# arkworks-rs/gemini

Measured on AMD Instinct MI355X. Metric: BLS12-381 G1 MSM throughput, higher is better.
Workload: dtype u32x12 Montgomery Fq (381-bit integer), u32x8 Fr; 1 GPU; 2^20 G1 MSM per GPU (BASELINE configs[1]: 2^20 G1 MSM on one MI355X); pairs_per_gpu=1048576

## Files before the change

### gemini_amd/capi.py

```python
from __future__ import annotations

import ctypes as C
import os

import numpy as np

_HERE = os.path.dirname(os.path.abspath(__file__))
LIB_PATH = os.environ.get("GM_LIB_PATH") or os.path.join(_HERE, "libgemini_hip.so")

GM_OK = 0
ERRORS = {-1: "GM_EINVAL", -2: "GM_ENOTINIT", -3: "GM_EHANDLE", -4: "GM_EHIP", -5: "GM_ENOMEM", -6: "GM_ESTATE"}

SYMBOLS = [
    "gm_init", "gm_shutdown", "gm_last_error", "gm_abi_version",
    "gm_g1_msm", "gm_g1_bases_register", "gm_g1_bases_free", "gm_g1_bases_len", "gm_g1_bases_download", "gm_g1_bases_precompute", "gm_set_auto_tables", "gm_g1_bases_table_info", "gm_pool_trim", "gm_g1_release_spare_tables", "gm_mem_stats", "gm_mem_reset_peak", "gm_runtime_info", "gm_snark_footprint", "gm_psnark_footprint", "gm_footprint_admit",
    "gm_g1_msm_h", "gm_g1_msm_v", "gm_g1_msm_v_batch", "gm_g1_msm_v_batch_partial", "gm_g1_msm_v_batch_at", "gm_g1_msm_d", "gm_g1_msm_d_partial", "gm_g1_sum",
    "gm_g1_msm_stream_new", "gm_g1_msm_stream_new_h", "gm_g1_msm_stream_add", "gm_g1_msm_stream_finalize", "gm_g1_msm_stream_free", "gm_host_alloc", "gm_host_free",
    "gm_g1_fixed_base_register", "gm_g1_srs_register", "gm_g1_srs_register_segments", "gm_set_msm_window", "gm_set_msm_table_min", "gm_set_msm_affine_levels", "gm_set_msm_split", "gm_set_msm_glv", "gm_set_msm_sort_group", "gm_debug_msm_sort_path", "gm_prof_enable", "gm_prof_read", "gm_prof_read_clock",
    "gm_idx_register", "gm_idx_free", "gm_idx_len", "gm_idx_download", "gm_idx_extend_frequency", "gm_fr_gather", "gm_fr_alg_hash", "gm_fr_plookup_set", "gm_fr_add_scalar", "gm_fr_shift_monic",
    "gm_fr_acc_product", "gm_fr_tensor_range", "gm_fr_tensor_gather", "gm_fr_powers_gather", "gm_fr_alg_hash_from", "gm_fr_powers_range", "gm_fr_plookup_set_block", "gm_fr_shift_block", "gm_fr_product", "gm_fr_acc_product_block",
    "gm_sc_set_shard_rounds", "gm_sc_round_begin_many", "gm_psnark_shard_block", "gm_psnark_shard_level", "gm_psnark_shard_footprint", "gm_psnark_shard_key_new", "gm_psnark_index_sharded", "gm_psnark_new_time_sharded", "gm_snark_new_elastic_sharded",
    "gm_fr_vec_alloc", "gm_fr_vec_free", "gm_fr_vec_len", "gm_fr_vec_upload", "gm_fr_vec_download",
    "gm_fr_vec_fill", "gm_fr_vec_ptr", "gm_fr_vec_set_len",
    "gm_fr_reverse", "gm_fr_stride", "gm_fr_fold", "gm_fr_fold_chain", "gm_fr_powers", "gm_fr_tensor", "gm_fr_hadamard", "gm_fr_ip", "gm_fr_eval_le", "gm_fr_eval_le_batch",
    "gm_fr_lincomb", "gm_fr_scale_into", "gm_fr_scale_into_many", "gm_fr_add_at", "gm_fr_div_vanishing",
    "gm_spm_register", "gm_spm_free", "gm_spm_mul", "gm_spm_shape", "gm_snark_new_time", "gm_snark_new_elastic", "gm_psnark_new_time", "gm_psnark_new_elastic", "gm_psnark_preprocess", "gm_psnark_preprocess_free", "gm_psnark_index", "gm_spm_download",
    "gm_sc_new", "gm_sc_new_v", "gm_sc_new_borrow", "gm_sc_round", "gm_sc_round_begin", "gm_sc_round_end", "gm_sc_fold", "gm_sc_rounds", "gm_sc_final", "gm_sc_free",
    "gm_sc_set_shard", "gm_sc_lens", "gm_sc_download",
    "gm_sp_new", "gm_sp_new_v", "gm_sp_new_borrow", "gm_sp_round", "gm_sp_fold", "gm_sp_rounds", "gm_sp_final", "gm_sp_to_time", "gm_sp_free",
    "gm_sc_set_herring", "gm_hg1_new", "gm_hg1_round", "gm_hg1_fold", "gm_hg1_rounds", "gm_hg1_final", "gm_hg1_free",
    "gm_g2_msm", "gm_g2_bases_register", "gm_g2_bases_free", "gm_g2_bases_len", "gm_g2_bases_download", "gm_g2_msm_h", "gm_g2_msm_v", "gm_g2_msm_d", "gm_g2_sum",
    "gm_hg2_new", "gm_hg2_round", "gm_hg2_fold", "gm_hg2_rounds", "gm_hg2_final", "gm_hg2_free",
    "gm_pairing_multi", "gm_pairing_multi_h", "gm_gt_mul", "gm_gt_pow", "gm_gt_one", "gm_gt_final_exp",
# ... 71 lines not shown
def ensure_init():
    if not _initialised:
        init()


MEM_FIELDS = ("device_total", "device_free", "held", "held_peak", "pool_cached", "in_use", "in_use_peak", "tables", "keys",
              "spare_table_releases", "msm_workspaces", "reserved")


def mem_stats() -> dict:
    out = np.zeros(12, dtype=np.uint64)
    check(load().gm_mem_stats(ptr(out)))
    return {k: int(v) for k, v in zip(MEM_FIELDS, out)}


FOOTPRINT_FIELDS = ("vectors", "workspaces_to_grow", "needed", "available")


def snark_footprint(ck_handle: int, num_constraints: int, elastic: bool = False) -> dict:
    out = np.zeros(4, dtype=np.uint64)
    check(load().gm_snark_footprint(C.c_uint64(ck_handle), C.c_size_t(num_constraints), C.c_int(int(elastic)), ptr(out)))
    return {k: int(v) for k, v in zip(FOOTPRINT_FIELDS, out)}


def psnark_footprint(ck_handle: int, num_variables: int, nnz: int, elastic: int = 0) -> dict:
    out = np.zeros(4, dtype=np.uint64)
    check(load().gm_psnark_footprint(C.c_uint64(ck_handle), C.c_size_t(num_variables), C.c_size_t(nnz), C.c_int(int(elastic)), ptr(out)))
    return {k: int(v) for k, v in zip(FOOTPRINT_FIELDS, out)}


# ... 25 lines not shown
```

### gemini_amd/csrc/capi.hip

```cpp
#include <cstring>
#include <vector>

#include "ctx.hpp"
#include "host_field.hpp"

namespace gm {

static thread_local char g_err[512] = "";
void set_error(const char* fmt, ...) {
  va_list ap;
  va_start(ap, fmt);
  vsnprintf(g_err, sizeof g_err, fmt, ap);
  va_end(ap);
}
int hip_fail(hipError_t e, const char* what, const char* file, int line) {
  set_error("HIP error %d (%s) in %s at %s:%d", (int)e, hipGetErrorString(e), what, file, line);
  return e == hipErrorOutOfMemory ? GM_ENOMEM : GM_EHIP;
}

MemStats& mem_stats() {
  static MemStats* m = new MemStats;
  return *m;
}
void MemStats::note_cached(ptrdiff_t delta) {
// ... 375 lines not shown
  for (auto& kv : C->provers) sc_destroy(kv.second.get());
  for (auto& kv : C->space_provers) sp_destroy(C, kv.second.get());
  for (auto& kv : C->herring) herring_destroy(C, kv.second.get());
  for (auto& kv : C->g2_bases)
    if (kv.second->d) (void)gm::raw_free(kv.second->d);
  for (auto& kv : C->crs) crs_destroy(kv.second.get());
  C->partial_bufs.release_all();
  for (auto& kv : C->indices)
    if (kv.second->d) (void)gm::raw_free(kv.second->d);
  for (auto& kv : C->matrices) {
    if (kv.second->rowptr) (void)gm::raw_free(kv.second->rowptr);
    if (kv.second->cols) (void)gm::raw_free(kv.second->cols);
    if (kv.second->vals) (void)gm::raw_free(kv.second->vals);
  }
  auto release_ws = [](MsmWorkspace& w) {
    for (DevBuf* b : {&w.scalars, &w.counts, &w.offsets, &w.cursor, &w.entries, &w.tmp_entries, &w.sortmeta, &w.buckets, &w.pk[0], &w.pk[1], &w.pp[0],
                      &w.pp[1], &w.rows, &w.cols, &w.planes, &w.misc, &w.lvl_cnt, &w.lvl_pos, &w.lvl_pts[0], &w.lvl_pts[1], &w.lvl_keys[0],
                      &w.lvl_keys[1], &w.lvl_prefix, &w.lvl_lane, &w.lvl_entries, &w.lvl_n})
      b->release();
    for (int k = 0; k < MSM_SLOTS; k++)
      if (w.host_planes[k]) (void)hipHostFree(w.host_planes[k]);
    if (w.have_done_ev) {
      for (int e = 0; e < MSM_SLOTS; e++) (void)hipEventDestroy(w.done_ev[e]);
    }
  };
  release_ws(C->msm);
  g2_workspace_release(C->g2);
  pairing_workspace_release(C->pairing);
  release_ws(C->msm_b);
  if (C->stream_b) (void)hipStreamDestroy(C->stream_b);
  for (int k = 0; k < MSM_SMALL_LANES; k++) {
// ... 280 lines not shown
           "gm_set_msm_sort_group: a block stages %zu .. %zu entries in its LDS (0 = the most), not %zu", MSM_SORT_GROUP_CAP_MIN, MSM_SORT_GROUP_CAP_MAX, cap);
  std::lock_guard<std::recursive_mutex> lk(C->msm_mu);
  C->msm_sort_group = mode;
  C->msm_sort_group_cap = cap;
  return GM_OK;
}

int gm_debug_msm_sort_path(int* out) {
  GM_CTX();
  GM_CHECK(out != nullptr, GM_EINVAL, "gm_debug_msm_sort_path: null output");
  std::lock_guard<std::recursive_mutex> lk(C->msm_mu);
  *out = C->msm_sort_path_last;
  return GM_OK;
}

int gm_set_msm_split(int on) {
  GM_CTX();
#ifndef GM_EXPERIMENTS
  GM_CHECK(on == 0, GM_EINVAL, "gm_set_msm_split: the window-group experiment is not in this build (make EXTRA=-DGM_EXPERIMENTS; DESIGN.md section 8)");
#endif
  C->msm_split = on != 0;
  return GM_OK;
}

int gm_set_msm_affine_levels(int levels) {
  GM_CTX();
  GM_CHECK(levels >= -1 && levels <= 8, GM_EINVAL, "gm_set_msm_affine_levels: %d not in [-1, 8]", levels);
#ifndef GM_EXPERIMENTS
  if (levels == -1) levels = 0;
  GM_CHECK(levels == 0, GM_EINVAL, "gm_set_msm_affine_levels: the affine-level experiment is not in this build (make EXTRA=-DGM_EXPERIMENTS; DESIGN.md section 8)");
// ... 1595 lines not shown
```

### gemini_amd/csrc/ctx.hpp

```cpp
#pragma once
#include <hip/hip_runtime.h>

#include <atomic>
#include <cstdarg>
#include <cstdint>
#include <cstdio>
#include <map>
#include <memory>
#include <mutex>
#include <string>
#include <unordered_map>
#include <vector>

#include "../../include/gemini_hip.h"

namespace gmh {
struct Fq12;
}

namespace gm {

void set_error(const char* fmt, ...);
int hip_fail(hipError_t e, const char* what, const char* file, int line);

// ... 162 lines not shown
};
struct MsmWorkspace;
constexpr size_t MSM_SORT_GROUP_CAP_MAX = (160 * 1024 - 3 * 1024 * 4 - 64) / 4;
constexpr size_t MSM_SORT_GROUP_CAP_MIN = 1024;
struct MsmPending {
  MsmWorkspace* ws = nullptr;
  int slot = 0;
  bool empty = true;
  int Wb = 0, c = 0, m = 0;
  uint32_t nbits = 0, wf[3] = {0, 0, 0};
  size_t plane_off[3] = {0, 0, 0};
  size_t plane_count = 0;
  int multi_levels = 0;
  int multi_W = 0;
  bool sort_compact = false;
};
struct MsmStreamSlot {
  uint8_t *raw = nullptr, *packed = nullptr, *scalars = nullptr;
  size_t raw_cap = 0, packed_cap = 0, scalars_cap = 0;
  hipEvent_t copied;
  bool have_ev = false;
  bool inflight = false;
  MsmPending P;
};
struct MsmStream {
  std::mutex mu;
  size_t chunk = 0, stride = 96;
  int mont = 0;
  uint64_t bases_handle = 0;
  int64_t base0 = 0, next_base = 0, step = 1;
  MsmStreamSlot s[2];
  int cur = 0;
  size_t fill = 0, total = 0;
  hipStream_t copy = nullptr;
  uint64_t acc[18];
  bool acc_set = false;
};

constexpr int MSM_SLOTS = 4;
constexpr int MSM_SMALL_LANES = 6;
struct MsmWorkspace {
  DevBuf scalars, counts, offsets, cursor, entries, tmp_entries, sortmeta, buckets, pk[2], pp[2], rows, cols, planes, misc;
  DevBuf clk;
  DevBuf lvl_cnt, lvl_pos, lvl_pts[2], lvl_keys[2], lvl_prefix, lvl_lane, lvl_entries, lvl_n;
  uint64_t* host_planes[MSM_SLOTS] = {};
  size_t host_planes_cap[MSM_SLOTS] = {};
  hipEvent_t done_ev[MSM_SLOTS];
  hipEvent_t sort_ev, acc_ev;
  bool have_done_ev = false;
};

enum ProfStage { PROF_DIGITS = 0, PROF_SCAN, PROF_SCATTER, PROF_ACC0, PROF_MERGE, PROF_REDUCE, PROF_SC_ROUND, PROF_EXTFREQ, PROF_NSTAGES };
struct Profiler {
  bool on = false;
  int only_stage = -1;
  hipEvent_t ev[2][2 * PROF_NSTAGES];
  bool have_events = false;
// ... 65 lines not shown
  DevBuf fr_scratch;
  uint64_t* host_small = nullptr;
  uint8_t* sc_desc_host = nullptr;
  uint8_t* sc_desc_dev = nullptr;
  hipEvent_t sc_desc_copied[SC_DESC_SLOTS] = {};
  unsigned sc_desc_next = 0;
  uint64_t* host_batch = nullptr;
  size_t host_batch_cap = 0;
  int msm_c_override = 0;
  int msm_glv = 0;
  int msm_split = 0;
  int msm_affine_levels = 0;
  int msm_sort_group = 1;
  size_t msm_sort_group_cap = 0;
  int msm_sort_path_last = 0;
  size_t msm_table_min = (size_t)1 << 17;
  int zero_copy = 3;
  std::atomic<int> msm_busy{0};
  bool auto_tables = true;
  size_t auto_tables_max = 0;
  int cu_count = 256;
};

Context* context();
struct MemStats {
  std::mutex mu;
  std::unordered_map<void*, size_t> sizes;
  size_t live = 0, peak_live = 0;
  size_t cached = 0;
  size_t peak_in_use = 0;
// ... 133 lines not shown
```

### gemini_amd/csrc/msm.hip

```cpp
#include <algorithm>
#include <atomic>
#include <chrono>
#include <condition_variable>
#include <cstdlib>
#include <cstring>
#include <functional>
#include <sched.h>
#include <cstdio>
#include <thread>
#include <vector>

#include "ctx.hpp"
#include "g1.cuh"
#include "host_field.hpp"

namespace gm {

constexpr uint32_t KEY_INV = 0xffffffffu;
constexpr int XYZZ_BYTES = 192;
constexpr int AFF_BYTES = 96;

struct DigitIter {
  uint32_t s[8];
  uint32_t carry;
// ... 1108 lines not shown

#ifdef GM_EXPERIMENTS
#include "msm_levels.inc"
#endif

__global__ __launch_bounds__(64) void k_merge(const uint32_t* __restrict__ keys_in, const uint8_t* __restrict__ pts_in,
                                              uint32_t E, uint32_t* __restrict__ keys_out,
                                              uint8_t* __restrict__ pts_out, uint8_t* __restrict__ buckets,
                                              int final_level) {
  __shared__ __attribute__((aligned(16))) uint8_t lds[128 * XYZZ30_BYTES];
  const int lane = threadIdx.x;
  const uint32_t wave = blockIdx.x;
  const uint32_t s0 = wave * 128u + 2u * lane;
  uint32_t hk = s0 < E ? keys_in[s0] : KEY_INV;
  uint32_t tk = s0 + 1 < E ? keys_in[s0 + 1] : KEY_INV;
  uint32_t hs = 2 * lane, ts = 2 * lane + 1;
  auto copy_rec = [](void* dst, const void* src) {
    const gm_u4v* s = reinterpret_cast<const gm_u4v*>(src);
    gm_u4v* d = reinterpret_cast<gm_u4v*>(dst);
#pragma unroll
    for (int i = 0; i < 13; i++) d[i] = s[i];
  };
  auto add_slots = [&](uint32_t dst_slot, uint32_t src_slot, Acc30& a) {
    Acc30 o;
    acc30_load(a, lds + dst_slot * XYZZ30_BYTES);
    acc30_load(o, lds + src_slot * XYZZ30_BYTES);
    acc30_add(a, o);
  };
  if (hk != KEY_INV) copy_rec(lds + hs * XYZZ30_BYTES, pts_in + (size_t)s0 * XYZZ30_BYTES);
  if (tk != KEY_INV) copy_rec(lds + ts * XYZZ30_BYTES, pts_in + ((size_t)s0 + 1) * XYZZ30_BYTES);
// ... 70 lines not shown
    __syncthreads();
  }
  if (lane == 0) {
    if (final_level) {
      if (hk != KEY_INV) copy_rec(buckets + (size_t)hk * XYZZ30_BYTES, lds + hs * XYZZ30_BYTES);
      if (tk != KEY_INV) copy_rec(buckets + (size_t)tk * XYZZ30_BYTES, lds + ts * XYZZ30_BYTES);
    } else {
      keys_out[2 * (size_t)wave] = hk;
      keys_out[2 * (size_t)wave + 1] = tk;
      if (hk != KEY_INV) copy_rec(pts_out + (size_t)(2 * (size_t)wave) * XYZZ30_BYTES, lds + hs * XYZZ30_BYTES);
      if (tk != KEY_INV) copy_rec(pts_out + (size_t)(2 * (size_t)wave + 1) * XYZZ30_BYTES, lds + ts * XYZZ30_BYTES);
    }
  }
}

enum { GS_STRIDED = 0, GS_PLANE = 1 };
struct GroupSumArgs {
  const uint8_t* in;
  uint8_t* out;
  int mode;
  uint32_t n_out;
  uint32_t per_win;
  uint32_t win_stride;
  uint32_t n_lo, s_hi, s_lo, s_e, len;
  uint32_t nb;
  uint32_t lpo_shift;
  int out_canonical;
  const uint32_t* in_cnt;
};
struct GroupSumJobs {
  GroupSumArgs j[3];
  uint32_t blk_end[3];
  const uint32_t* err_src;
  uint32_t* err_dst;
  const unsigned long long* clk_src;
  const uint32_t* chunked_src;
};

__global__ __launch_bounds__(256) void k_group_sum(GroupSumJobs J) {
  if (J.err_dst && blockIdx.x == 0 && threadIdx.x == 0) {
    *J.err_dst = *J.err_src;
    J.err_dst[1] = J.chunked_src ? *J.chunked_src : 0u;
    if (J.clk_src) {
      unsigned long long* d = reinterpret_cast<unsigned long long*>(J.err_dst + 2);
      d[0] = J.clk_src[0];
      d[1] = J.clk_src[1];
    }
  }
  const int job = blockIdx.x < J.blk_end[0] ? 0 : (blockIdx.x < J.blk_end[1] ? 1 : 2);
  const GroupSumArgs& a = J.j[job];
  const uint32_t blk0 = job == 0 ? 0u : J.blk_end[job - 1];
  const uint8_t* __restrict__ in = a.in;
  uint8_t* __restrict__ out = a.out;
  const uint32_t gt = (blockIdx.x - blk0) * blockDim.x + threadIdx.x;
  const uint32_t lpo = 1u << a.lpo_shift;
  const uint32_t o = gt >> a.lpo_shift, q = gt & (lpo - 1u);
  Acc30 acc;
  acc30_zero(acc);
  const uint32_t* __restrict__ in_cnt = a.in_cnt;
  auto filled = [&](size_t slot) { return in_cnt == nullptr || in_cnt[slot] != 0u; };
  auto add_rec = [&](size_t slot) {
    if (!filled(slot)) return;
// ... 220 lines not shown
  static const size_t c20_min = getenv("GM_MSM_C20_MIN") ? (size_t)strtoull(getenv("GM_MSM_C20_MIN"), nullptr, 10) : ((size_t)7 << 21);
  if (n >= c20_min) return 20;
  if (lg >= 23) return 19;
  static const int c_medium = getenv("GM_MSM_C_MEDIUM") ? atoi(getenv("GM_MSM_C_MEDIUM")) : 0;
  if (c_medium && lg >= 14 && lg <= 17) return c_medium;
  if (lg >= 14) return 16;
  if (lg >= 11) return 8;
  if (lg >= 8) return lg - 4;
  if (lg >= 5) return lg + 1;
  return 4;
}

size_t msm_workspace_held(const MsmWorkspace& ws) {
  size_t b = 0;
  for (const DevBuf* d : {&ws.scalars, &ws.counts, &ws.offsets, &ws.cursor, &ws.entries, &ws.tmp_entries, &ws.sortmeta, &ws.buckets, &ws.pk[0], &ws.pk[1],
                          &ws.pp[0], &ws.pp[1], &ws.rows, &ws.cols, &ws.planes, &ws.misc, &ws.clk})
    b += d->cap;
  return b;
}
size_t msm_workspace_bound(Context* C, const Bases* bases, size_t n) {
  if (n == 0) return 0;
  n = std::min<size_t>(n, (size_t)1 << 26);
  int c = C->msm_c_override ? C->msm_c_override : choose_window(n);
  bool table = false;
  if (bases && !C->msm_c_override && n < ((size_t)1 << ENTRY_W_SHIFT)) {
    if (bases->table && n >= std::max(C->msm_table_min, bases->tab_min)) {
      c = bases->tab_c;
      table = true;
    } else {
      for (const Bases::TableSet& ts : bases->extra)
        if (n >= ts.min_n && n < ts.max_n && n <= ts.n) {
          c = ts.c;
          table = true;
          break;
        }
    }
  }
  const size_t W = (size_t)(256 + c - 1) / (size_t)c;
  const size_t N = n * W, nbuckets = (table ? 1 : W) << (c - 1);
  auto grow = [](size_t b) { return b + b / 8 + 256; };
  const size_t lanes0 = N >= ((size_t)1 << 24) ? 262144 : 131072;
  const size_t L = std::min<size_t>(256, std::max<size_t>(4, (N + lanes0 - 1) / lanes0)) + 1;
  const size_t E1 = 2 * ((N / L + 256 + 255) / 256 * 256), E2 = 2 * ((E1 + 127) / 128);
  size_t b = 2 * grow(N * 8);
  b += grow(nbuckets * XYZZ30_BYTES) + 4 * grow((nbuckets + 8192) * 4);
  b += grow(E1 * 4) + grow(E1 * XYZZ30_BYTES) + grow(E2 * 4) + grow(E2 * XYZZ30_BYTES);
  b += (size_t)W * ((size_t)3 << 14) * XYZZ30_BYTES + ((size_t)16 << 20);
  return b;
}

constexpr size_t MSM_SMALL_N = (size_t)1 << 17;
constexpr size_t MSM_SPLIT_MIN_N = (size_t)1 << 17;
static int msm_run_one(Context* C, const Bases* bases, int64_t first, int64_t step, const void* d_scalars, int mont, size_t n,
                       bool normalize, uint64_t out_jac[18]);

struct MsmStreams {
  hipStream_t sort, acc, tail;
};
struct MsmMulti {
  bool block = false;
  int levels = 0;
// ... 451 lines not shown
  uint64_t Nacc = N;
  for (int l = 0; l < levels; l++) Nacc = Nacc / 2 + 2 * nbuckets + 2;

  static const int L_env = getenv("GM_MSM_L") ? atoi(getenv("GM_MSM_L")) : 0;
  const uint64_t Nacc_all = nparts > 1 ? Nall : Nacc;
  const uint64_t lanes0 = Nacc_all >= ((uint64_t)1 << 24) ? 262144 : 131072;
  static const uint64_t L_cap = getenv("GM_MSM_LCAP") ? (uint64_t)atoi(getenv("GM_MSM_LCAP")) : 256;
  uint32_t L = (uint32_t)std::min<uint64_t>(L_cap, std::max<uint64_t>(4, (Nacc_all + lanes0 - 1) / lanes0));
  if (L_env > 0) L = (uint32_t)L_env;
  L = (L + 1u) & ~1u;
  const uint64_t T0 = (Nacc + L - 1) / L;
  const uint64_t T0pad = (T0 + 255) / 256 * 256;
  const uint64_t E1 = 2 * T0pad;

  int rc;
  const size_t counts_words = (nbuckets + 2 + SORT_GMAX + 2 + 63) / 64 * 64;
  if ((rc = ws.counts.ensure(counts_words * 4))) return rc;
  if ((rc = ws.offsets.ensure((nbuckets + 1) * 4))) return rc;
  if ((rc = ws.cursor.ensure((nbuckets + 1) * 4))) return rc;
  if ((rc = ws.misc.ensure((nbuckets / SCAN_PER_BLOCK + 2) * 4))) return rc;
  if ((rc = ws.entries.ensure(N * 8))) return rc;
  if ((rc = ws.buckets.ensure(nbuckets * bucket_bytes))) return rc;
  if ((rc = ws.pk[0].ensure(E1 * 4))) return rc;
  if ((rc = ws.pp[0].ensure(E1 * bucket_bytes))) return rc;
  const uint64_t E2 = 2 * ((E1 + 127) / 128);
  if ((rc = ws.pk[1].ensure(E2 * 4))) return rc;
  if ((rc = ws.pp[1].ensure(E2 * bucket_bytes))) return rc;

  const uint32_t* sc = reinterpret_cast<const uint32_t*>(d_scalars);
  GM_HIP(hipMemsetAsync(ws.counts.p, 0, counts_words * 4, st));
  uint32_t* d_err = ws.counts.as<uint32_t>() + nbuckets + 1;
  uint32_t* d_chunked = ws.counts.as<uint32_t>() + nbuckets + 2 + SORT_GMAX + 1;
  const bool bucket_counts_valid = levels == 0;
  if (!bucket_counts_valid) GM_HIP(hipMemsetAsync(ws.buckets.p, 0, nbuckets * bucket_bytes, st));
  const uint32_t dblocks = (uint32_t)((n + 255) / 256);
  Profiler& pf = C->prof;
  auto run_scan = [&]() {
    const uint32_t nb = (uint32_t)((nbuckets + SCAN_PER_BLOCK - 1) / SCAN_PER_BLOCK);
    hipLaunchKernelGGL(k_scan_block_sums, dim3(nb), dim3(256), 0, st, ws.counts.as<uint32_t>(), (uint32_t)nbuckets,
                       ws.misc.as<uint32_t>());
    hipLaunchKernelGGL(k_scan_top, dim3(1), dim3(1024), 0, st, ws.misc.as<uint32_t>(), nb,
                       ws.offsets.as<uint32_t>() + nbuckets);
    hipLaunchKernelGGL(k_scan_apply, dim3(nb), dim3(256), 0, st, ws.counts.as<uint32_t>(), (uint32_t)nbuckets,
                       ws.misc.as<uint32_t>(), ws.offsets.as<uint32_t>(), ws.cursor.as<uint32_t>());
  };
  static const bool sort_atomic_env = getenv("GM_MSM_SORT") && !strcmp(getenv("GM_MSM_SORT"), "atomic");
  static const bool sort_flat_env = !(getenv("GM_MSM_SORT") && !strcmp(getenv("GM_MSM_SORT"), "blocks"));
// ... 178 lines not shown
                       acc_tab, L, ws.pk[0].as<uint32_t>(), ws.pp[0].as<uint8_t>(), ws.buckets.as<uint8_t>(), use_glv ? bases->phi : (const uint8_t*)nullptr, acc_clk);
  else if (acc0_waves == 2)
    hipLaunchKernelGGL(k_acc0<2>, dim3((uint32_t)(T0pad / 256)), dim3(256), acc0_lds_pad, st, acc_entries, acc_total, acc_bases, acc_first, acc_step,
                       acc_tab, L, ws.pk[0].as<uint32_t>(), ws.pp[0].as<uint8_t>(), ws.buckets.as<uint8_t>(), use_glv ? bases->phi : (const uint8_t*)nullptr, acc_clk);
  else
    hipLaunchKernelGGL(k_acc0<3>, dim3((uint32_t)(T0pad / 256)), dim3(256), 0, st, acc_entries, acc_total, acc_bases, acc_first, acc_step,
                       acc_tab, L, ws.pk[0].as<uint32_t>(), ws.pp[0].as<uint8_t>(), ws.buckets.as<uint8_t>(), use_glv ? bases->phi : (const uint8_t*)nullptr, acc_clk);
  pf.end(part, PROF_ACC0, st);
  if (sts.tail != st) {
    GM_HIP(hipEventRecord(ws.acc_ev, st));
    GM_HIP(hipStreamWaitEvent(sts.tail, ws.acc_ev, 0));
  }
  st = sts.tail;
  pf.begin(part, PROF_MERGE, st);
  {
    uint64_t E = E1;
    int src = 0;
    for (;;) {
      uint32_t waves = (uint32_t)((E + 127) / 128);
      int final_level = waves == 1;
      hipLaunchKernelGGL(k_merge, dim3(waves), dim3(64), 0, st, ws.pk[src].as<uint32_t>(), ws.pp[src].as<uint8_t>(),
                         (uint32_t)E, ws.pk[src ^ 1].as<uint32_t>(), ws.pp[src ^ 1].as<uint8_t>(),
                         ws.buckets.as<uint8_t>(), final_level);
      if (final_level) break;
      E = 2ull * waves;
      src ^= 1;
    }
  }

  pf.end(part, PROF_MERGE, st);
  pf.begin(part, PROF_REDUCE, st);
  const uint32_t nbits = (uint32_t)(c - 1);
  uint32_t wf[3] = {0, 0, 0};
  int m;
  static const int fields_env = getenv("GM_MSM_FIELDS") ? atoi(getenv("GM_MSM_FIELDS")) : 0;
  if (nbits <= 7) {
    m = 1;
    wf[0] = nbits;
  } else if (nbits <= 14 || (fields_env == 2 && nbits <= 16)) {
    m = 2;
    wf[0] = nbits / 2;
// ... 28 lines not shown
    g.in = in; g.out = out; g.mode = GS_PLANE; g.out_canonical = 1;
    g.in_cnt = in == bucket_in ? bucket_cnt : nullptr;
    g.per_win = nb + 1; g.n_out = (uint32_t)Wb * g.per_win; g.win_stride = 1u << nb; g.nb = nb;
    g.lpo_shift = lpo_for(nb ? (1u << (nb - 1)) : 1u, g.n_out);
    return g;
  };
  uint8_t* planes = nullptr;
  size_t plane_count = 0;
  auto launch = [&](std::initializer_list<GroupSumArgs> jobs, bool last = false) {
    GroupSumJobs J{};
    if (last) {
      J.err_src = d_err;
      J.err_dst = reinterpret_cast<uint32_t*>(planes + plane_count * XYZZ_BYTES);
      J.clk_src = ws.clk.as<unsigned long long>();
      J.chunked_src = d_chunked;
    }
    uint32_t tot = 0;
    int k = 0;
    for (const GroupSumArgs& g : jobs) {
      J.j[k] = g;
      tot += (uint32_t)((((uint64_t)g.n_out << g.lpo_shift) + 255) / 256);
      J.blk_end[k] = tot;
      k++;
    }
    for (; k < 3; k++) J.blk_end[k] = tot;
    hipLaunchKernelGGL(k_group_sum, dim3(tot), dim3(256), 0, st, J);
  };
  size_t plane_off[3];
  for (int k = 0; k < m; k++) {
    plane_off[k] = plane_count;
    plane_count += (size_t)Wb * (wf[k] + 1);
  }
  const size_t plane_bytes = plane_count * XYZZ_BYTES + 24;
  if (ws.host_planes_cap[slot] < plane_bytes) {
    if (ws.host_planes[slot]) (void)hipHostFree(ws.host_planes[slot]);
    ws.host_planes[slot] = nullptr;
    ws.host_planes_cap[slot] = 0;
    GM_HIP(hipHostMalloc((void**)&ws.host_planes[slot], plane_bytes, hipHostMallocDefault));
    ws.host_planes_cap[slot] = plane_bytes;
  }
  const bool zc = (C->zero_copy & 2) != 0;
  if (zc) {
    planes = reinterpret_cast<uint8_t*>(ws.host_planes[slot]);
  } else {
    if ((rc = ws.planes.ensure(plane_count * XYZZ_BYTES + 64))) return rc;
    planes = ws.planes.as<uint8_t>();
  }
  const uint8_t* X = ws.buckets.as<uint8_t>();
// ... 20 lines not shown
    launch({strided(X, A, B, n2, n1, n1 * n0, n0, 1, n0), strided(X, Bm, B, n2, n0, n1 * n0, 1, n0, n1)});
    lpo_jobs = 3;
    launch({strided(A, Y2, n2 * n1, 1, n2, 0, n1, 1, n1), strided(A, Y1, n2 * n1, 1, n1, 0, 1, n1, n2),
            strided(Bm, Y0, n2 * n0, 1, n0, 0, 1, n0, n2)});
    launch({plane(Y0, planes + plane_off[0] * XYZZ_BYTES, wf[0]), plane(Y1, planes + plane_off[1] * XYZZ_BYTES, wf[1]),
            plane(Y2, planes + plane_off[2] * XYZZ_BYTES, wf[2])}, true);
  }
  pf.end(part, PROF_REDUCE, st);
  GM_HIP(hipGetLastError());
  if (!zc) GM_HIP(hipMemcpyAsync(ws.host_planes[slot], planes, plane_bytes, hipMemcpyDeviceToHost, st));
  GM_HIP(hipEventRecord(ws.done_ev[slot], st));
  P->Wb = Wb;
  P->multi_levels = multi ? multi->levels : 0;
  P->multi_W = multi ? (use_table ? 1 : W) : 0;
  P->plane_count = plane_count;
  P->c = c;
  P->m = m;
  P->nbits = nbits;
  for (int k = 0; k < 3; k++) {
    P->wf[k] = wf[k];
    P->plane_off[k] = k < m ? plane_off[k] : 0;
  }
  return GM_OK;
}

class HornerPool {
 public:
  static HornerPool& get() {
    static HornerPool p;
    return p;
// ... 119 lines not shown

static void horner_pool_prewake() { HornerPool::get().prewake(); }
static void horner_pool_run(int n, const std::function<void(int)>& fn) { HornerPool::get().run(n, fn); }

static int msm_finish_parts(Context* C, const MsmPending* parts, int nparts, bool normalize, uint64_t out_jac[18], bool use_pool, uint64_t* const* multi_out) {
  gmh::G1 result = gmh::G1::identity();
  int rc = GM_OK;
  for (int p = nparts - 1; p >= 0; p--) {
    const MsmPending& P = parts[p];
    if (P.empty) continue;
    MsmWorkspace& ws = *P.ws;
    if (P.Wb > 1 && use_pool) HornerPool::get().prewake();
    GM_HIP(hipEventSynchronize(ws.done_ev[P.slot]));
    const uint64_t* hp = ws.host_planes[P.slot];
    C->msm_sort_path_last = P.sort_compact ? 1 + (int)((hp[P.plane_count * 24] >> 32) != 0) : 0;
    if ((uint32_t)hp[P.plane_count * 24] != 0) {
      set_error("msm: a scalar passed as a canonical integer is >= 2^255 (not the BigInt image of an Fr element)");
      rc = GM_EINVAL;
      continue;
    }
    if (rc) continue;
    auto plane_at = [&](int w, int field, uint32_t j) {
      return gmh::xyzz_to_jac_dev(hp + (P.plane_off[field] + (size_t)w * (P.wf[field] + 1) + j) * 24);
    };
    std::vector<gmh::G1> S((size_t)P.Wb);
    auto window_sum = [&](int w) {
      gmh::G1 s = gmh::G1::identity();
      int field = P.m - 1;
      uint32_t jj = P.wf[field];
      for (int j = (int)P.nbits - 1; j >= 0; j--) {
// ... 487 lines not shown
```

### include/gemini_hip.h

```cpp
#ifndef GEMINI_HIP_H
#define GEMINI_HIP_H

#include <stddef.h>
#include <stdint.h>

#ifdef __cplusplus
extern "C" {
#endif

#define GM_OK 0
#define GM_EINVAL (-1)
#define GM_ENOTINIT (-2)
#define GM_EHANDLE (-3)
#define GM_EHIP (-4)
#define GM_ENOMEM (-5)
#define GM_ESTATE (-6)

int gm_init(int device);
void gm_shutdown(void);
const char* gm_last_error(void);
int gm_abi_version(void);

int gm_g1_msm(const void* bases, size_t base_stride, const uint64_t* scalars, size_t n, uint64_t out_jac[18]);

// ... 40 lines not shown
int gm_g1_msm_stream_finalize(uint64_t stream, uint64_t out_jac[18], size_t* pairs_or_null);
int gm_g1_msm_stream_free(uint64_t stream);
int gm_host_alloc(size_t bytes, void** p);
int gm_host_free(void* p);

int gm_g1_fixed_base_register(const uint64_t base_affine[12], const uint64_t* scalars, size_t n, uint64_t* handle);
int gm_g1_srs_register(const uint64_t base_affine[12], const uint64_t tau[4], size_t n, uint64_t* handle);
int gm_g1_srs_register_segments(const uint64_t base_affine[12], const uint64_t tau[4], const size_t* starts, const size_t* counts, size_t nseg,
                                uint64_t* handle);

int gm_set_msm_window(int c);
int gm_set_msm_table_min(size_t n);
int gm_set_msm_glv(int on);
int gm_set_msm_sort_group(int mode, size_t cap);
int gm_debug_msm_sort_path(int* out);
int gm_set_msm_split(int on);
int gm_set_msm_affine_levels(int levels);

#define GM_PROF_NSTAGES 8
int gm_prof_enable(int on);
int gm_prof_read(double* ms_out, uint64_t* count_out, int n);
int gm_prof_read_clock(double* acc0_mhz);

int gm_fr_vec_alloc(size_t n, uint64_t* handle);
int gm_fr_vec_free(uint64_t handle);
int gm_fr_vec_len(uint64_t handle, size_t* n);
int gm_fr_vec_upload(uint64_t handle, size_t offset, const uint64_t* mont, size_t n);
int gm_fr_vec_download(uint64_t handle, size_t offset, uint64_t* mont, size_t n);
int gm_fr_vec_fill(uint64_t handle, const uint64_t value_mont[4]);
int gm_fr_vec_ptr(uint64_t handle, void** dptr);
// ... 389 lines not shown
```

### include/gemini_hip.hpp

```cpp
#pragma once
#include <array>
#include <cstdint>
#include <cstring>
#include <map>
#include <optional>
#include <stdexcept>
#include <string>
#include <utility>
#include <vector>

#include "gemini_hip.h"

namespace gm {

struct Error : std::runtime_error {
  int code;
  Error(int c, const std::string& m) : std::runtime_error(m), code(c) {}
};
inline void check(int rc) {
  if (rc != GM_OK) throw Error(rc, gm_last_error());
}
inline void init(int device = 0) { check(gm_init(device)); }
inline void release_spare_tables() { check(gm_g1_release_spare_tables()); }
struct MemStats {
  uint64_t device_total, device_free, held, held_peak, pool_cached, in_use, in_use_peak, tables, keys, spare_table_releases, msm_workspaces, reserved;
};
inline MemStats mem_stats() {
  uint64_t v[12];
  check(gm_mem_stats(v));
  return MemStats{v[0], v[1], v[2], v[3], v[4], v[5], v[6], v[7], v[8], v[9], v[10], v[11]};
}
inline void mem_reset_peak() { check(gm_mem_reset_peak()); }
struct Footprint {
  uint64_t vectors, workspaces_to_grow, needed, available;
};
inline Footprint snark_footprint(uint64_t ck_handle, size_t num_constraints, bool elastic = false) {
  uint64_t v[4];
  check(gm_snark_footprint(ck_handle, num_constraints, elastic ? 1 : 0, v));
  return Footprint{v[0], v[1], v[2], v[3]};
}
inline Footprint psnark_footprint(uint64_t ck_handle, size_t num_variables, size_t nnz, int elastic = 0) {
  uint64_t v[4];
  check(gm_psnark_footprint(ck_handle, num_variables, nnz, elastic, v));
  return Footprint{v[0], v[1], v[2], v[3]};
}

inline size_t psnark_shard_block(size_t longest, int world) { return gm_psnark_shard_block(longest, world); }
// ... 1531 lines not shown
```

Measured before the change: 357.2 Mscalar/s.

## Add opt-in boundary pre-pass and empty-wave early exit to MSM merge tree

Adds an optional k_boundary kernel, off by default and enabled through gm_set_msm_boundary. Before the merge tree, it resolves each lane's head and tail keys that are already complete: it copies them straight into buckets, adds adjacent tail/head pairs that share a key, and writes the remaining keys to a new bk buffer for the first merge level. Separately, k_merge now returns early for any wave whose keys are all invalid, which always applies. Stats (pairs added, slots copied, slots left) travel back through the group-sum error area into a debug query. The costs are an extra key buffer, an extra kernel launch when enabled, and more host-plane bytes.

Result: no change. 358.9 Mscalar/s (median of 2 runs) (+0.5%).

```diff
diff --git a/gemini_amd/capi.py b/gemini_amd/capi.py
--- a/gemini_amd/capi.py
+++ b/gemini_amd/capi.py
@@ -16,7 +16,7 @@
     "gm_g1_msm", "gm_g1_bases_register", "gm_g1_bases_free", "gm_g1_bases_len", "gm_g1_bases_download", "gm_g1_bases_precompute", "gm_set_auto_tables", "gm_g1_bases_table_info", "gm_pool_trim", "gm_g1_release_spare_tables", "gm_mem_stats", "gm_mem_reset_peak", "gm_runtime_info", "gm_snark_footprint", "gm_psnark_footprint", "gm_footprint_admit",
     "gm_g1_msm_h", "gm_g1_msm_v", "gm_g1_msm_v_batch", "gm_g1_msm_v_batch_partial", "gm_g1_msm_v_batch_at", "gm_g1_msm_d", "gm_g1_msm_d_partial", "gm_g1_sum",
     "gm_g1_msm_stream_new", "gm_g1_msm_stream_new_h", "gm_g1_msm_stream_add", "gm_g1_msm_stream_finalize", "gm_g1_msm_stream_free", "gm_host_alloc", "gm_host_free",
-    "gm_g1_fixed_base_register", "gm_g1_srs_register", "gm_g1_srs_register_segments", "gm_set_msm_window", "gm_set_msm_table_min", "gm_set_msm_affine_levels", "gm_set_msm_split", "gm_set_msm_glv", "gm_set_msm_sort_group", "gm_debug_msm_sort_path", "gm_prof_enable", "gm_prof_read", "gm_prof_read_clock",
+    "gm_g1_fixed_base_register", "gm_g1_srs_register", "gm_g1_srs_register_segments", "gm_set_msm_window", "gm_set_msm_table_min", "gm_set_msm_affine_levels", "gm_set_msm_split", "gm_set_msm_glv", "gm_set_msm_sort_group", "gm_debug_msm_sort_path", "gm_set_msm_boundary", "gm_debug_msm_tail", "gm_prof_enable", "gm_prof_read", "gm_prof_read_clock",
     "gm_idx_register", "gm_idx_free", "gm_idx_len", "gm_idx_download", "gm_idx_extend_frequency", "gm_fr_gather", "gm_fr_alg_hash", "gm_fr_plookup_set", "gm_fr_add_scalar", "gm_fr_shift_monic",
     "gm_fr_acc_product", "gm_fr_tensor_range", "gm_fr_tensor_gather", "gm_fr_powers_gather", "gm_fr_alg_hash_from", "gm_fr_powers_range", "gm_fr_plookup_set_block", "gm_fr_shift_block", "gm_fr_product", "gm_fr_acc_product_block",
     "gm_sc_set_shard_rounds", "gm_sc_round_begin_many", "gm_psnark_shard_block", "gm_psnark_shard_level", "gm_psnark_shard_footprint", "gm_psnark_shard_key_new", "gm_psnark_index_sharded", "gm_psnark_new_time_sharded", "gm_snark_new_elastic_sharded",
@@ -118,6 +118,19 @@
     return {k: int(v) for k, v in zip(MEM_FIELDS, out)}
 
 
+MSM_TAIL_FIELDS = ("chunk_len", "lanes", "pairs_added", "slots_copied", "slots_left")
+
+
+def set_msm_boundary(on: int):
+    check(load().gm_set_msm_boundary(C.c_int(on)))
+
+
+def msm_tail() -> dict:
+    out = np.zeros(5, dtype=np.uint64)
+    check(load().gm_debug_msm_tail(ptr(out)))
+    return {k: int(v) for k, v in zip(MSM_TAIL_FIELDS, out)}
+
+
 FOOTPRINT_FIELDS = ("vectors", "workspaces_to_grow", "needed", "available")
 
 
diff --git a/gemini_amd/csrc/capi.hip b/gemini_amd/csrc/capi.hip
--- a/gemini_amd/csrc/capi.hip
+++ b/gemini_amd/csrc/capi.hip
@@ -413,7 +413,7 @@
     if (kv.second->vals) (void)gm::raw_free(kv.second->vals);
   }
   auto release_ws = [](MsmWorkspace& w) {
-    for (DevBuf* b : {&w.scalars, &w.counts, &w.offsets, &w.cursor, &w.entries, &w.tmp_entries, &w.sortmeta, &w.buckets, &w.pk[0], &w.pk[1], &w.pp[0],
+    for (DevBuf* b : {&w.scalars, &w.counts, &w.offsets, &w.cursor, &w.entries, &w.tmp_entries, &w.sortmeta, &w.buckets, &w.pk[0], &w.pk[1], &w.bk, &w.pp[0],
                       &w.pp[1], &w.rows, &w.cols, &w.planes, &w.misc, &w.lvl_cnt, &w.lvl_pos, &w.lvl_pts[0], &w.lvl_pts[1], &w.lvl_keys[0],
                       &w.lvl_keys[1], &w.lvl_prefix, &w.lvl_lane, &w.lvl_entries, &w.lvl_n})
       b->release();
@@ -724,6 +724,22 @@
   return GM_OK;
 }
 
+int gm_set_msm_boundary(int on) {
+  GM_CTX();
+  GM_CHECK(on == 0 || on == 1, GM_EINVAL, "gm_set_msm_boundary: on = %d not in {0, 1}", on);
+  std::lock_guard<std::recursive_mutex> lk(C->msm_mu);
+  C->msm_boundary = on;
+  return GM_OK;
+}
+
+int gm_debug_msm_tail(uint64_t out[5]) {
+  GM_CTX();
+  GM_CHECK(out != nullptr, GM_EINVAL, "gm_debug_msm_tail: null output");
+  std::lock_guard<std::recursive_mutex> lk(C->msm_mu);
+  for (int i = 0; i < 5; i++) out[i] = C->msm_tail_last[i];
+  return GM_OK;
+}
+
 int gm_set_msm_split(int on) {
   GM_CTX();
 #ifndef GM_EXPERIMENTS
diff --git a/gemini_amd/csrc/ctx.hpp b/gemini_amd/csrc/ctx.hpp
--- a/gemini_amd/csrc/ctx.hpp
+++ b/gemini_amd/csrc/ctx.hpp
@@ -200,6 +200,8 @@
   int multi_levels = 0;
   int multi_W = 0;
   bool sort_compact = false;
+  uint32_t L = 0;
+  uint64_t T0 = 0;
 };
 struct MsmStreamSlot {
   uint8_t *raw = nullptr, *packed = nullptr, *scalars = nullptr;
@@ -227,6 +229,7 @@
 constexpr int MSM_SMALL_LANES = 6;
 struct MsmWorkspace {
   DevBuf scalars, counts, offsets, cursor, entries, tmp_entries, sortmeta, buckets, pk[2], pp[2], rows, cols, planes, misc;
+  DevBuf bk;
   DevBuf clk;
   DevBuf lvl_cnt, lvl_pos, lvl_pts[2], lvl_keys[2], lvl_prefix, lvl_lane, lvl_entries, lvl_n;
   uint64_t* host_planes[MSM_SLOTS] = {};
@@ -322,6 +325,8 @@
   int msm_sort_group = 1;
   size_t msm_sort_group_cap = 0;
   int msm_sort_path_last = 0;
+  int msm_boundary = 0;
+  uint64_t msm_tail_last[5] = {0, 0, 0, 0, 0};
   size_t msm_table_min = (size_t)1 << 17;
   int zero_copy = 3;
   std::atomic<int> msm_busy{0};
diff --git a/gemini_amd/csrc/msm.hip b/gemini_amd/csrc/msm.hip
--- a/gemini_amd/csrc/msm.hip
+++ b/gemini_amd/csrc/msm.hip
@@ -1146,6 +1146,13 @@
   const uint32_t s0 = wave * 128u + 2u * lane;
   uint32_t hk = s0 < E ? keys_in[s0] : KEY_INV;
   uint32_t tk = s0 + 1 < E ? keys_in[s0 + 1] : KEY_INV;
+  if (!__any(hk != KEY_INV || tk != KEY_INV)) {
+    if (lane == 0 && !final_level) {
+      keys_out[2 * (size_t)wave] = KEY_INV;
+      keys_out[2 * (size_t)wave + 1] = KEY_INV;
+    }
+    return;
+  }
   uint32_t hs = 2 * lane, ts = 2 * lane + 1;
   auto copy_rec = [](void* dst, const void* src) {
     const gm_u4v* s = reinterpret_cast<const gm_u4v*>(src);
@@ -1246,6 +1253,53 @@
   }
 }
 
+__global__ __launch_bounds__(256) __attribute__((amdgpu_waves_per_eu(2, 2))) void k_boundary(const uint32_t* __restrict__ keys_in,
+                                                                                             const uint8_t* __restrict__ pts, uint32_t T,
+                                                                                             uint32_t* __restrict__ keys_out,
+                                                                                             uint8_t* __restrict__ buckets,
+                                                                                             uint32_t* __restrict__ stat) {
+  const uint32_t t = blockIdx.x * blockDim.x + threadIdx.x;
+  const uint2 mine = reinterpret_cast<const uint2*>(keys_in)[t];
+  const uint32_t hk = mine.x, tk = mine.y;
+  const bool has_next = t + 1 < T;
+  const uint2 next = has_next ? reinterpret_cast<const uint2*>(keys_in)[t + 1] : make_uint2(KEY_INV, KEY_INV);
+  const uint2 prev = t > 0 ? reinterpret_cast<const uint2*>(keys_in)[t - 1] : make_uint2(KEY_INV, KEY_INV);
+  const uint32_t prev_last = prev.y != KEY_INV ? prev.y : prev.x;
+  const bool two = tk != KEY_INV;
+  const bool pair = two && has_next && next.y != KEY_INV && next.x == tk;
+  const bool taken = two && t > 0 && prev.y != KEY_INV && prev.y == hk;
+  const bool tail_done = two && (!has_next || next.x != tk);
+  const bool head_done = two && (t == 0 || prev_last != hk);
+  auto copy_rec = [](void* dst, const void* src) {
+    const gm_u4v* s = reinterpret_cast<const gm_u4v*>(src);
+    gm_u4v* d = reinterpret_cast<gm_u4v*>(dst);
+#pragma unroll
+    for (int i = 0; i < 13; i++) d[i] = s[i];
+  };
+  if (head_done) copy_rec(buckets + (size_t)hk * XYZZ30_BYTES, pts + (size_t)(2 * (size_t)t) * XYZZ30_BYTES);
+  if (tail_done) copy_rec(buckets + (size_t)tk * XYZZ30_BYTES, pts + (size_t)(2 * (size_t)t + 1) * XYZZ30_BYTES);
+  if (__any(pair)) {
+    if (pair) {
+      Acc30 a, o;
+      acc30_load(a, pts + (size_t)(2 * (size_t)t + 1) * XYZZ30_BYTES);
+      acc30_load(o, pts + (size_t)(2 * (size_t)t + 2) * XYZZ30_BYTES);
+      acc30_add(a, o);
+      acc30_store(buckets + (size_t)tk * XYZZ30_BYTES, a);
+    }
+  }
+  const bool keep_h = hk != KEY_INV && !head_done && !taken;
+  const bool keep_t = two && !tail_done && !pair;
+  reinterpret_cast<uint2*>(keys_out)[t] = make_uint2(keep_h ? hk : KEY_INV, keep_t ? tk : KEY_INV);
+  const uint32_t n_pair = (uint32_t)__popcll(__ballot(pair));
+  const uint32_t n_copy = (uint32_t)(__popcll(__ballot(head_done)) + __popcll(__ballot(tail_done)));
+  const uint32_t n_left = (uint32_t)(__popcll(__ballot(keep_h)) + __popcll(__ballot(keep_t)));
+  if ((threadIdx.x & 63u) == 0) {
+    if (n_pair) atomicAdd(stat, n_pair);
+    if (n_copy) atomicAdd(stat + 1, n_copy);
+    if (n_left) atomicAdd(stat + 2, n_left);
+  }
+}
+
 enum { GS_STRIDED = 0, GS_PLANE = 1 };
 struct GroupSumArgs {
   const uint8_t* in;
@@ -1267,6 +1321,7 @@
   uint32_t* err_dst;
   const unsigned long long* clk_src;
   const uint32_t* chunked_src;
+  const uint32_t* tail_src;
 };
 
 __global__ __launch_bounds__(256) void k_group_sum(GroupSumJobs J) {
@@ -1278,6 +1333,7 @@
       d[0] = J.clk_src[0];
       d[1] = J.clk_src[1];
     }
+    for (int i = 0; i < 3; i++) J.err_dst[6 + i] = J.tail_src ? J.tail_src[i] : 0u;
   }
   const int job = blockIdx.x < J.blk_end[0] ? 0 : (blockIdx.x < J.blk_end[1] ? 1 : 2);
   const GroupSumArgs& a = J.j[job];
@@ -1528,7 +1584,7 @@
 size_t msm_workspace_held(const MsmWorkspace& ws) {
   size_t b = 0;
   for (const DevBuf* d : {&ws.scalars, &ws.counts, &ws.offsets, &ws.cursor, &ws.entries, &ws.tmp_entries, &ws.sortmeta, &ws.buckets, &ws.pk[0], &ws.pk[1],
-                          &ws.pp[0], &ws.pp[1], &ws.rows, &ws.cols, &ws.planes, &ws.misc, &ws.clk})
+                          &ws.bk, &ws.pp[0], &ws.pp[1], &ws.rows, &ws.cols, &ws.planes, &ws.misc, &ws.clk})
     b += d->cap;
   return b;
 }
@@ -1559,6 +1615,7 @@
   size_t b = 2 * grow(N * 8);
   b += grow(nbuckets * XYZZ30_BYTES) + 4 * grow((nbuckets + 8192) * 4);
   b += grow(E1 * 4) + grow(E1 * XYZZ30_BYTES) + grow(E2 * 4) + grow(E2 * XYZZ30_BYTES);
+  b += grow(E1 * 4);
   b += (size_t)W * ((size_t)3 << 14) * XYZZ30_BYTES + ((size_t)16 << 20);
   return b;
 }
@@ -2040,7 +2097,7 @@
   const uint64_t E1 = 2 * T0pad;
 
   int rc;
-  const size_t counts_words = (nbuckets + 2 + SORT_GMAX + 2 + 63) / 64 * 64;
+  const size_t counts_words = (nbuckets + 2 + SORT_GMAX + 5 + 63) / 64 * 64;
   if ((rc = ws.counts.ensure(counts_words * 4))) return rc;
   if ((rc = ws.offsets.ensure((nbuckets + 1) * 4))) return rc;
   if ((rc = ws.cursor.ensure((nbuckets + 1) * 4))) return rc;
@@ -2052,11 +2109,14 @@
   const uint64_t E2 = 2 * ((E1 + 127) / 128);
   if ((rc = ws.pk[1].ensure(E2 * 4))) return rc;
   if ((rc = ws.pp[1].ensure(E2 * bucket_bytes))) return rc;
+  const bool boundary = C->msm_boundary != 0;
+  if (boundary && (rc = ws.bk.ensure(E1 * 4))) return rc;
 
   const uint32_t* sc = reinterpret_cast<const uint32_t*>(d_scalars);
   GM_HIP(hipMemsetAsync(ws.counts.p, 0, counts_words * 4, st));
   uint32_t* d_err = ws.counts.as<uint32_t>() + nbuckets + 1;
   uint32_t* d_chunked = ws.counts.as<uint32_t>() + nbuckets + 2 + SORT_GMAX + 1;
+  uint32_t* d_tail = d_chunked + 1;
   const bool bucket_counts_valid = levels == 0;
   if (!bucket_counts_valid) GM_HIP(hipMemsetAsync(ws.buckets.p, 0, nbuckets * bucket_bytes, st));
   const uint32_t dblocks = (uint32_t)((n + 255) / 256);
@@ -2265,17 +2325,22 @@
   st = sts.tail;
   pf.begin(part, PROF_MERGE, st);
   {
+    if (boundary)
+      hipLaunchKernelGGL(k_boundary, dim3((uint32_t)(T0pad / 256)), dim3(256), 0, st, ws.pk[0].as<uint32_t>(), ws.pp[0].as<uint8_t>(), (uint32_t)T0pad,
+                         ws.bk.as<uint32_t>(), ws.buckets.as<uint8_t>(), d_tail);
     uint64_t E = E1;
     int src = 0;
+    const uint32_t* keys = boundary ? ws.bk.as<uint32_t>() : ws.pk[0].as<uint32_t>();
     for (;;) {
       uint32_t waves = (uint32_t)((E + 127) / 128);
       int final_level = waves == 1;
-      hipLaunchKernelGGL(k_merge, dim3(waves), dim3(64), 0, st, ws.pk[src].as<uint32_t>(), ws.pp[src].as<uint8_t>(),
+      hipLaunchKernelGGL(k_merge, dim3(waves), dim3(64), 0, st, keys, ws.pp[src].as<uint8_t>(),
                          (uint32_t)E, ws.pk[src ^ 1].as<uint32_t>(), ws.pp[src ^ 1].as<uint8_t>(),
                          ws.buckets.as<uint8_t>(), final_level);
       if (final_level) break;
       E = 2ull * waves;
       src ^= 1;
+      keys = ws.pk[src].as<uint32_t>();
     }
   }
 
@@ -2334,6 +2399,7 @@
       J.err_dst = reinterpret_cast<uint32_t*>(planes + plane_count * XYZZ_BYTES);
       J.clk_src = ws.clk.as<unsigned long long>();
       J.chunked_src = d_chunked;
+      J.tail_src = d_tail;
     }
     uint32_t tot = 0;
     int k = 0;
@@ -2351,7 +2417,7 @@
     plane_off[k] = plane_count;
     plane_count += (size_t)Wb * (wf[k] + 1);
   }
-  const size_t plane_bytes = plane_count * XYZZ_BYTES + 24;
+  const size_t plane_bytes = plane_count * XYZZ_BYTES + 40;
   if (ws.host_planes_cap[slot] < plane_bytes) {
     if (ws.host_planes[slot]) (void)hipHostFree(ws.host_planes[slot]);
     ws.host_planes[slot] = nullptr;
@@ -2402,6 +2468,8 @@
   P->multi_levels = multi ? multi->levels : 0;
   P->multi_W = multi ? (use_table ? 1 : W) : 0;
   P->plane_count = plane_count;
+  P->L = L;
+  P->T0 = T0;
   P->c = c;
   P->m = m;
   P->nbits = nbits;
@@ -2551,6 +2619,14 @@
     GM_HIP(hipEventSynchronize(ws.done_ev[P.slot]));
     const uint64_t* hp = ws.host_planes[P.slot];
     C->msm_sort_path_last = P.sort_compact ? 1 + (int)((hp[P.plane_count * 24] >> 32) != 0) : 0;
+    if (use_pool) {
+      const uint32_t* tw = reinterpret_cast<const uint32_t*>(hp + P.plane_count * 24) + 6;
+      uint64_t* o = C->msm_tail_last;
+      if (p == nparts - 1) o[1] = o[2] = o[3] = o[4] = 0;
+      o[0] = P.L;
+      o[1] += P.T0;
+      for (int i = 0; i < 3; i++) o[2 + i] += tw[i];
+    }
     if ((uint32_t)hp[P.plane_count * 24] != 0) {
       set_error("msm: a scalar passed as a canonical integer is >= 2^255 (not the BigInt image of an Fr element)");
       rc = GM_EINVAL;
diff --git a/include/gemini_hip.h b/include/gemini_hip.h
--- a/include/gemini_hip.h
+++ b/include/gemini_hip.h
@@ -78,6 +78,8 @@
 int gm_set_msm_glv(int on);
 int gm_set_msm_sort_group(int mode, size_t cap);
 int gm_debug_msm_sort_path(int* out);
+int gm_set_msm_boundary(int on);
+int gm_debug_msm_tail(uint64_t out[5]);
 int gm_set_msm_split(int on);
 int gm_set_msm_affine_levels(int levels);
 
diff --git a/include/gemini_hip.hpp b/include/gemini_hip.hpp
--- a/include/gemini_hip.hpp
+++ b/include/gemini_hip.hpp
@@ -31,6 +31,15 @@
   return MemStats{v[0], v[1], v[2], v[3], v[4], v[5], v[6], v[7], v[8], v[9], v[10], v[11]};
 }
 inline void mem_reset_peak() { check(gm_mem_reset_peak()); }
+struct MsmTail {
+  uint64_t chunk_len, lanes, pairs_added, slots_copied, slots_left;
+};
+inline void set_msm_boundary(bool on) { check(gm_set_msm_boundary(on ? 1 : 0)); }
+inline MsmTail msm_tail() {
+  uint64_t v[5];
+  check(gm_debug_msm_tail(v));
+  return MsmTail{v[0], v[1], v[2], v[3], v[4]};
+}
 struct Footprint {
   uint64_t vectors, workspaces_to_grow, needed, available;
 };
```
